# cielavenir/7bgzf

Measured on AMD Instinct MI355X. Metric: GB/s input compressed, BGZF 64KiB blocks, higher is better.
Workload: dtype u8

## Files before the change

### 7bgzf_amd/__init__.py

```python
import ctypes
import os

import numpy as np

HERE = os.path.dirname(os.path.abspath(__file__))
LIB_PATH = os.path.join(HERE, "libhipdeflate.so")

FRAME_RAW, FRAME_BGZF, FRAME_MIGZ, FRAME_RAW_FLUSH, FRAME_ZLIB, FRAME_GZIP = 0, 1, 2, 3, 4, 5
FRAME_LATENCY = 0x100
DEFLATE_HIP = 11
HD_E_NODEVICE, HD_E_ARG, HD_E_NOMEM = 100, 101, 102

BGZF_BLOCK = 0xff00
WG_LEVEL = 3
BGZF_EOF = bytes.fromhex("1f8b08040000000000ff0600424302001b0003000000000000000000")


class HipDeflateError(RuntimeError):
    pass


_lib = None
_vp = ctypes.c_void_p


class MemberSummary(ctypes.Structure):
    _fields_ = [("nmembers", ctypes.c_uint64), ("out_bytes", ctypes.c_uint64), ("end_offset", ctypes.c_uint64),
                ("status", ctypes.c_uint32)]


class RangeSummary(ctypes.Structure):
    _fields_ = [("out_bytes", ctypes.c_uint64), ("nselected", ctypes.c_uint64), ("sel_bytes", ctypes.c_uint64),
                ("nrefused", ctypes.c_uint64), ("bad_member", ctypes.c_uint64), ("status", ctypes.c_uint32)]


RANGE_BYTES, RANGE_VOFFSET = 0, 1
RANGE_PIECE = 256 << 10


def voffset(coffset, uoffset):
    return (int(coffset) << 16) | (int(uoffset) & 0xffff)


EXPORTS = [
    "hipdeflate_init", "hipdeflate_shutdown", "hipdeflate_available", "hipdeflate_version", "hipdeflate_stall_count",
    "hip_deflate", "hip_deflate_flush", "hip_inflate", "hipdeflate_batch_deflate", "hipdeflate_batch_inflate",
    "hipdeflate_batch_deflate_dev", "hipdeflate_batch_inflate_dev", "hipdeflate_scan_sizes_dev",
    "hipdeflate_compact_dev", "hipdeflate_scratch_bytes", "bgzf_compress", "hipdeflate_selftest",
    "hipdeflate_pipe_open", "hipdeflate_pipe_input", "hipdeflate_pipe_submit", "hipdeflate_pipe_result",
    "hipdeflate_pipe_close", "hipdeflate_unpipe_open", "hipdeflate_unpipe_input", "hipdeflate_unpipe_submit",
    "hipdeflate_unpipe_result", "hipdeflate_unpipe_close", "hipdeflate_test_build_lengths", "hipdeflate_test_beside",
    "hip_inflate_flush", "hipdeflate_batch_inflate_flush", "hipdeflate_batch_inflate_flush_dev", "hipdeflate_bound",
    "hipdeflate_compact_span_dev", "hipdeflate_index_members_dev", "hipdeflate_verify_members_dev",
    "hipdeflate_read_ranges_dev",
    "hipdeflate_init_devices", "hipdeflate_device_count", "hipdeflate_use_device",
    "hipdeflate_pipe_open_on", "hipdeflate_unpipe_open_on", "hipdeflate_lat_open_on",
    "hipdeflate_pipe_members", "hipdeflate_lat_open", "hipdeflate_lat_input", "hipdeflate_lat_run", "hipdeflate_lat_output", "hipdeflate_lat_close",
]


def _link_hip_runtime():
    import importlib.util
    spec = importlib.util.find_spec("torch")
    link = os.path.join(HERE, "hiprt", "libamdhip64.so.7")
    target = None
    if spec is not None and spec.submodule_search_locations:
        cand = os.path.join(list(spec.submodule_search_locations)[0], "lib", "libamdhip64.so")
        if os.path.exists(cand):
            target = cand
    try:
        if target is None:
            if os.path.islink(link) or os.path.exists(link):
                os.remove(link)
        elif not (os.path.islink(link) and os.readlink(link) == target):
            os.makedirs(os.path.dirname(link), exist_ok=True)
            if os.path.islink(link) or os.path.exists(link):
                os.remove(link)
            os.symlink(target, link)
    except OSError:
        pass


def lib():
    global _lib
# ... 41 lines not shown
                                               ctypes.POINTER(MemberSummary), _vp]
    L.hipdeflate_verify_members_dev.argtypes = [_vp, _vp, _vp, _vp, _vp, ctypes.c_uint32, ctypes.POINTER(ctypes.c_uint64), _vp]
    L.hipdeflate_read_ranges_dev.argtypes = [_vp, _vp, _vp, _vp, _vp, _vp, ctypes.c_uint32, ctypes.c_int, _vp, _vp, ctypes.c_uint32,
                                             _vp, ctypes.c_uint64, _vp, _vp, _vp, ctypes.POINTER(RangeSummary), _vp]
    L.hipdeflate_pipe_open.restype = _vp
    L.hipdeflate_pipe_open.argtypes = [ctypes.c_int, ctypes.c_int, ctypes.c_uint32, ctypes.c_uint32, ctypes.c_int]
    L.hipdeflate_pipe_input.restype = _vp
    L.hipdeflate_pipe_input.argtypes = [_vp, sz_p]
    L.hipdeflate_pipe_submit.argtypes = [_vp, ctypes.c_size_t]
    L.hipdeflate_pipe_result.argtypes = [_vp, ctypes.POINTER(_vp), sz_p, ctypes.POINTER(ctypes.c_uint32)]
    L.hipdeflate_pipe_members.argtypes = [_vp, ctypes.POINTER(_vp), ctypes.POINTER(_vp), ctypes.POINTER(_vp)]
    L.hipdeflate_pipe_close.restype = None
    L.hipdeflate_pipe_close.argtypes = [_vp]
    L.hipdeflate_unpipe_open.restype = _vp
    L.hipdeflate_unpipe_open.argtypes = [ctypes.c_uint32, ctypes.c_size_t, ctypes.c_size_t, ctypes.c_int]
    L.hipdeflate_unpipe_input.restype = _vp
    L.hipdeflate_unpipe_input.argtypes = [_vp, sz_p]
    L.hipdeflate_unpipe_submit.argtypes = [_vp, _vp, _vp, _vp, ctypes.c_uint32]
    L.hipdeflate_unpipe_result.argtypes = [_vp, ctypes.POINTER(_vp), sz_p]
    L.hipdeflate_unpipe_close.restype = None
    L.hipdeflate_unpipe_close.argtypes = [_vp]
    L.hipdeflate_lat_open.restype = _vp
    L.hipdeflate_lat_open.argtypes = [ctypes.c_int, ctypes.c_int, ctypes.c_uint32, ctypes.c_uint32]
    L.hipdeflate_lat_input.restype = _vp
    L.hipdeflate_lat_input.argtypes = [_vp, ctypes.c_uint32]
    L.hipdeflate_lat_run.argtypes = [_vp, _vp, ctypes.c_uint32]
    L.hipdeflate_lat_output.restype = _vp
    L.hipdeflate_lat_output.argtypes = [_vp, ctypes.c_uint32, _vp, _vp, _vp]
    L.hipdeflate_lat_close.restype = None
    L.hipdeflate_lat_close.argtypes = [_vp]
    L.hipdeflate_test_build_lengths.argtypes = [_vp, ctypes.c_uint32, ctypes.c_uint32, ctypes.c_uint32, _vp]
    L.hipdeflate_test_beside.argtypes = [ctypes.c_int, ctypes.c_uint32]
    L.hipdeflate_test_beside.restype = None
    _lib = L
    return L


def _check(rc, what):
    if rc:
        raise HipDeflateError("%s failed with %d%s" % (
            what, rc, " (no usable gfx950 device; there is no CPU fallback)" if rc == HD_E_NODEVICE else ""))


def available():
    return lib().hipdeflate_available() == 0


def version():
    lib().hipdeflate_available()
    return lib().hipdeflate_version().decode()


def _np(a, dtype):
    return np.ascontiguousarray(a, dtype=dtype)


def _p(a):
    return a.ctypes.data_as(_vp)


def as_u8(data):
    if isinstance(data, np.ndarray):
        return np.ascontiguousarray(data, dtype=np.uint8)
    return np.frombuffer(bytes(data), dtype=np.uint8) if len(data) else np.zeros(0, dtype=np.uint8)


# ... 223 lines not shown
```

### 7bgzf_amd/csrc/hd_api.hip

```cpp
#include <hip/hip_runtime.h>
#include <stdio.h>
#include <stdlib.h>
#include <string.h>
#include <linux/futex.h>
#include <sys/syscall.h>
#include <unistd.h>
#include <sched.h>
#include <chrono>
#include <condition_variable>
#include <mutex>
#include <vector>

#include "../../include/hipdeflate.h"
#include "hd_deflate_static.hpp"
#include "hd_deflate_dynamic.hpp"
#include "hd_deflate_wg.hpp"
#include "hd_emit_wg.hpp"
#include "hd_inflate.hpp"
#include "hd_inflate_lat.hpp"
#include "hd_compact.hpp"
#include "hd_index.hpp"
#include "hd_range.hpp"
#include "hd_segment.hpp"

// ... 58 lines not shown
		const int r = reserve(n);
		if (r) {
			p = old;
			cap = old_cap;
			return r;
		}
		if (old)
			retired.push_back(old);
		return r;
	}
};

struct Ctx {
	bool ready = false;
	int failed = 0;
	int device = -1;
	char desc[256] = "hipdeflate (not initialised)";
	hipStream_t stream = nullptr;
	CrcTables *d_ct = nullptr;
	uint32_t *d_stalls = nullptr;
	std::mutex mu;
	Buf d_in, d_meta, d_slots, d_packed, d_scratch, d_scan;
	Buf h_in{ nullptr, 0, true }, h_meta{ nullptr, 0, true }, h_out{ nullptr, 0, true };
	std::mutex mu_dev;
	Buf d_tok;
	Buf d_tiles;
	hipEvent_t ev_tok = nullptr;
	hipStream_t st_tok = nullptr;
	bool tok_used = false;
	hd::WgBeside beside;
	hipEvent_t ev_tiles = nullptr;
	hipStream_t st_tiles = nullptr;
	bool tiles_used = false;
	std::mutex mu_index;
	Buf d_index, d_cand;
	Buf d_range, d_range_out;
};

constexpr int HD_MAX_CTX = 32;
Ctx g_all[HD_MAX_CTX];
int g_want[HD_MAX_CTX];
int g_nctx = 0;
thread_local int t_cur = 0;
std::mutex g_init_mu;
inline Ctx &cur() { return g_all[t_cur]; }

}
int hd_probe_lds_order(void);
namespace {
constexpr int CODEC_LEVELS = 13;
constexpr size_t CODEC_POOL_MAX = 64;
std::mutex g_codec_mu;
std::vector<hipdeflate_lat *> g_codec_free[CODEC_LEVELS];
void codec_pool_drain()
{
	std::lock_guard<std::mutex> lk(g_codec_mu);
	for (std::vector<hipdeflate_lat *> &f : g_codec_free) {
		for (hipdeflate_lat *c : f)
			hipdeflate_lat_close(c);
		f.clear();
	}
}

void build_crc_tables(CrcTables *t)
{
	const uint32_t poly = 0xEDB88320u;
// ... 138 lines not shown
	stamp();
	if (e != hipSuccess || ndev == 0) {
		fprintf(stderr, "hipdeflate: no HIP device (%s); there is no CPU fallback\n",
			e == hipSuccess ? "device count 0" : hipGetErrorString(e));
		return g.failed = HD_E_NODEVICE;
	}
	if (device < 0) {
		const char *s = getenv("HIPDEFLATE_DEVICE");
		if (!s || !*s)
			s = getenv("LOCAL_RANK");
		device = s && *s ? atoi(s) % ndev : 0;
	}
	if (device >= ndev)
		device = device % ndev;
	hipDeviceProp_t prop;
	HD_CHECK(hipSetDevice(device));
	HD_CHECK(hipGetDeviceProperties(&prop, device));
	if (strncmp(prop.gcnArchName, "gfx950", 6) != 0) {
		fprintf(stderr, "hipdeflate: device %d is %s; this library holds gfx950 (MI355X) code only\n", device,
			prop.gcnArchName);
		return g.failed = HD_E_NODEVICE;
	}
	stamp();
	HD_CHECK(hipStreamCreateWithFlags(&g.stream, hipStreamNonBlocking));
	stamp();
	CrcTables *h = (CrcTables *)malloc(sizeof(CrcTables));
	build_crc_tables(h);
	stamp();
	HD_CHECK(hipMalloc((void **)&g.d_ct, sizeof(CrcTables)));
	HD_CHECK(hipMemcpy(g.d_ct, h, sizeof(CrcTables), hipMemcpyHostToDevice));
	free(h);
	HD_CHECK(hipMalloc((void **)&g.d_stalls, 16));
	HD_CHECK(hipMemset(g.d_stalls, 0, 16));
	stamp();
	if (const int bad = hd_probe_lds_order()) {
		fprintf(stderr, "hipdeflate: device %d failed the LDS store-order probe (%d); this build's encoders are not "
			"reproducible on it and refuse to run\n", device, bad);
		(void)hipFree(g.d_ct);
		g.d_ct = nullptr;
		(void)hipFree(g.d_stalls);
		g.d_stalls = nullptr;
		(void)hipStreamDestroy(g.stream);
		g.stream = nullptr;
		return g.failed = HD_E_NODEVICE;
	}
	stamp();
	if (trace && nts == 7)
		fprintf(stderr, "hipdeflate init (ms): runtime + device count %.1f, set device + properties %.1f, stream %.1f, CRC tables on the CPU %.1f, "
			"first allocations + copy %.1f, first kernel (code object load + LDS order probe) %.1f; total %.1f\n",
			ts[1] - ts[0], ts[2] - ts[1], ts[3] - ts[2], ts[4] - ts[3], ts[5] - ts[4], ts[6] - ts[5], ts[6] - ts[0]);
	g.device = device;
	snprintf(g.desc, sizeof(g.desc), "hipdeflate 0.2 on device %d: %s (%s), %d CUs, %.0f GiB", device, prop.name,
		 prop.gcnArchName, prop.multiProcessorCount, prop.totalGlobalMem / 1073741824.0);
	g.ready = true;
	return 0;
}

inline int ensure_ctx(int idx)
{
	Ctx &g = g_all[idx];
	if (g.ready)
		return 0;
	{
		std::lock_guard<std::mutex> lk(g_init_mu);
		configure_locked(nullptr, 0);
		if (idx >= g_nctx)
			return HD_E_ARG;
	}
	return ctx_init(g, g_want[idx]);
}
inline int ensure() { return ensure_ctx(t_cur); }

inline int bind_device(const Ctx &g)
{
	HD_CHECK(hipSetDevice(g.device));
	return 0;
}
inline int bind_device() { return bind_device(cur()); }

struct OnCtx {
	int keep;
	explicit OnCtx(int idx) : keep(t_cur) { t_cur = idx; }
	~OnCtx() { t_cur = keep; }
};

static int code_batch(const hd::DeflateArgs &a, int level, hipStream_t st)
{
	if (level <= 1) {
		hd::DeflateArgs b = a;
		b.level = level;
		if (a.seg_slots)
			hipLaunchKernelGGL((hd::k_deflate_static<HD_L1_WIN_BITS, HD_L1_HASH_BITS, false, 0, true>), dim3(a.nblocks),
					   dim3(64), 0, st, b);
		else
			hipLaunchKernelGGL((hd::k_deflate_static<HD_L1_WIN_BITS, HD_L1_HASH_BITS, false>), dim3(a.nblocks), dim3(64), 0, st, b);
		return 0;
	}
	return hd::launch_deflate_dynamic(a, level, st);
}

int launch_deflate(const hd::DeflateArgs &a, int level, hipStream_t st)
{
	if (a.nblocks == 0)
		return 0;
	int r = a.seg_limit
			? hd::launch_deflate_segmented(a, level, st, [&](const hd::DeflateArgs &x) { return code_batch(x, level, st); })
			: code_batch(a, level, st);
	if (r)
		return r;
	if (a.frame == HD_FRAME_ZLIB)
		hipLaunchKernelGGL(hd::k_adler32_patch, dim3(a.nblocks), dim3(64), 0, st, a.in, a.in_off, a.in_len, a.nblocks,
				   a.out, a.out_stride, a.out_len, a.status);
	HD_CHECK(hipGetLastError());
	return 0;
}

inline size_t up16(size_t v) { return (v + 15) & ~(size_t)15; }

}

extern "C" {

int hipdeflate_init(int device)
{
	{
		std::lock_guard<std::mutex> lk(g_init_mu);
		if (device < 0)
			configure_locked(nullptr, 0);
		else
			configure_locked(&device, 1);
	}
	return ensure();
}

int hipdeflate_init_devices(const int *devices, int n)
{
	if (!devices || n < 1 || n > HD_MAX_CTX)
// ... 44 lines not shown
		Ctx &g = g_all[i];
		if (!g.ready || !g.d_stalls)
			continue;
		uint32_t v = 0;
		if (hipSetDevice(g.device) == hipSuccess && hipDeviceSynchronize() == hipSuccess &&
		    hipMemcpy(&v, g.d_stalls, 4, hipMemcpyDeviceToHost) == hipSuccess)
			sum += v;
	}
	return sum;
}

const char *hipdeflate_version(void) { return cur().desc; }

static void infb_drain();

void hipdeflate_shutdown(void)
{
	codec_pool_drain();
	infb_drain();
	std::lock_guard<std::mutex> lk(g_init_mu);
	for (int i = 0; i < HD_MAX_CTX; i++) {
		Ctx &g = g_all[i];
		g.failed = 0;
		if (!g.ready)
			continue;
		(void)hipSetDevice(g.device);
		(void)hipDeviceSynchronize();
		for (Buf *b : { &g.d_in, &g.d_meta, &g.d_slots, &g.d_packed, &g.d_scratch, &g.d_scan, &g.h_in, &g.h_meta,
				&g.h_out, &g.d_tok, &g.d_tiles, &g.d_index, &g.d_cand, &g.d_range, &g.d_range_out })
			b->release();
		(void)hipFree(g.d_ct);
		(void)hipFree(g.d_stalls);
		g.d_stalls = nullptr;
		(void)hipStreamDestroy(g.stream);
		if (g.ev_tok)
			(void)hipEventDestroy(g.ev_tok);
		if (g.ev_tiles)
			(void)hipEventDestroy(g.ev_tiles);
		g.ev_tok = g.ev_tiles = nullptr;
		g.beside.release();
		g.st_tok = g.st_tiles = nullptr;
		g.tok_used = g.tiles_used = false;
		g.d_ct = nullptr;
		g.stream = nullptr;
		g.ready = false;
	}
	g_nctx = 0;
}

static uint64_t scratch_need(uint32_t nblocks, uint32_t cap, int level, bool latency)
{
	if (level >= 1 && level < HD_WG_LEVEL && latency && cap > HD_LAT_SEG_BYTES(level))
		return hd::segmented_scratch_bytes(nblocks, cap, level, HD_LAT_SEG_BYTES(level));
	if (level >= 1 && level < HD_WG_LEVEL && cap > HD_SEG_LIMIT)
		return hd::segmented_scratch_bytes(nblocks, cap, level);
	return level < 2 ? 0 : hd::dynamic_scratch_bytes(nblocks, cap, level, 0, latency);
}

uint64_t hipdeflate_scratch_bytes(uint32_t nblocks, uint32_t max_block, int level)
{
	return scratch_need(nblocks, max_block, level, false);
}

uint64_t hipdeflate_bound(uint64_t block_bytes, int level)
{
	const uint32_t lat = HD_LAT_SEG_BYTES(level);
// ... 46 lines not shown
	a.skip_small = 0;
	a.split_max = hd::split_max_block(out_stride, out_cap);
	a.split_ovf = nullptr;
	const uint32_t seg_lim = latency ? HD_LAT_SEG_BYTES(level) : HD_SEG_LIMIT;
	a.seg_bytes = latency ? HD_LAT_SEG_BYTES(level) : HD_SEG_BYTES;
	a.seg_limit = (level >= 1 && level < HD_WG_LEVEL && a.split_max > seg_lim) ? seg_lim : 0;
	if (level >= HD_WG_LEVEL && max_in)
		a.split_max = max_in;
	a.lat = (latency && level >= HD_WG_LEVEL && a.split_max <= hd::EW_BLOCK_MAX) ? 1u : 0u;
	a.stalls = g.d_stalls;
	a.hint = 0;
	a.host_seg_off = nullptr;
	a.host_seg_len = nullptr;
	const uint64_t need = scratch_need(nblocks, a.split_max, level, latency);
	if (need) {
		std::lock_guard<std::mutex> lk(g.mu_dev);
		bool beside_fits = true;
		if (g.d_tok.grow_keep_old(need)) {
			const uint64_t extra = (level >= HD_WG_LEVEL && !a.lat) ? hd::wg_beside_bytes(nblocks, a.split_max) : 0;
			if (!extra || extra >= need || g.d_tok.grow_keep_old(need - extra))
				return HD_E_NOMEM;
			beside_fits = false;
		}
		a.scratch = (uint8_t *)g.d_tok.p;
		if (!g.ev_tok)
			HD_CHECK(hipEventCreateWithFlags(&g.ev_tok, hipEventDisableTiming));
		if (g.tok_used && g.st_tok != (hipStream_t)stream)
			HD_CHECK(hipStreamWaitEvent((hipStream_t)stream, g.ev_tok, 0));
		if (level >= HD_WG_LEVEL && !a.lat && beside_fits && beside_allowed() && g.beside.init() == 0) {
			a.beside = &g.beside;
			const uint32_t keep = (HD_WG_WAYS(level) == 4 && a.split_max <= 65536) ? 2u : 3u;
			a.beside_keep = g_test_beside_keep < keep ? g_test_beside_keep : keep;
		}
		r = launch_deflate(a, level, (hipStream_t)stream);
		if (!r) {
			HD_CHECK(hipEventRecord(g.ev_tok, (hipStream_t)stream));
			g.st_tok = (hipStream_t)stream;
			g.tok_used = true;
		}
		return r;
	}
	return launch_deflate(a, level, (hipStream_t)stream);
}

int hipdeflate_batch_deflate_dev(const void *in, const void *in_off, const void *in_len, uint32_t nblocks, int level,
				 int frame, void *out, uint64_t out_stride, uint32_t out_cap, void *out_len,
				 void *crc32, void *status, void *stream)
{
	return batch_deflate_dev_impl(in, in_off, in_len, nblocks, level, frame, out, out_stride, out_cap, out_len, crc32, status,
				      stream, 0);
}

static int batch_inflate_dev(const void *in, const void *in_off, const void *in_len, uint32_t nblocks, void *out,
			     const void *out_off, const void *out_cap, void *out_len, void *crc32, void *status, void *stream,
			     uint32_t flags)
{
	Ctx &g = cur();
	int r = ensure();
	if (r)
		return r;
	if (!out_len)
		return HD_E_ARG;
	if (nblocks == 0)
		return 0;
	hd::InflateArgs a;
	a.in = (const uint8_t *)in;
	a.in_off = (const uint64_t *)in_off;
	a.in_len = (const uint32_t *)in_len;
	a.nblocks = nblocks;
	a.out = (uint8_t *)out;
	a.out_off = (const uint64_t *)out_off;
	a.out_cap = (const uint32_t *)out_cap;
	a.out_len = (uint32_t *)out_len;
	a.crc = (uint32_t *)crc32;
	a.status = (int32_t *)status;
// ... 25 lines not shown
	Ctx &g = cur();
	int r = ensure();
	if (r)
		return r;
	if (nblocks == 0) {
		if (total)
			HD_CHECK(hipMemsetAsync(total, 0, 8, (hipStream_t)stream));
		return 0;
	}
	const uint32_t ntiles = (nblocks + hd::SCAN_TILE - 1) / hd::SCAN_TILE;
	std::lock_guard<std::mutex> lk(g.mu_dev);
	if (g.d_tiles.grow_keep_old((size_t)ntiles * 8))
		return HD_E_NOMEM;
	uint64_t *tiles = (uint64_t *)g.d_tiles.p;
	hipStream_t st = (hipStream_t)stream;
	if (!g.ev_tiles)
		HD_CHECK(hipEventCreateWithFlags(&g.ev_tiles, hipEventDisableTiming));
	if (g.tiles_used && g.st_tiles != st)
		HD_CHECK(hipStreamWaitEvent(st, g.ev_tiles, 0));
	hipLaunchKernelGGL(hd::k_scan_tile_sums, dim3(ntiles), dim3(256), 0, st, (const uint32_t *)out_len, nblocks, tiles);
	hipLaunchKernelGGL(hd::k_scan_tiles, dim3(1), dim3(256), 0, st, tiles, ntiles, base, (uint64_t *)total);
	hipLaunchKernelGGL(hd::k_scan_finish, dim3(ntiles), dim3(256), 0, st, (const uint32_t *)out_len, nblocks, tiles,
			   (uint64_t *)dst_off);
	HD_CHECK(hipGetLastError());
	HD_CHECK(hipEventRecord(g.ev_tiles, st));
	g.st_tiles = st;
	g.tiles_used = true;
	return 0;
}

int hipdeflate_compact_dev(const void *slots, uint64_t stride, const void *out_len, const void *dst_off,
			   uint32_t nblocks, void *dst, void *stream)
{
	int r = ensure();
	if (r)
		return r;
	if (nblocks == 0)
		return 0;
	if ((stride & 3) || ((uintptr_t)slots & 3))
		return HD_E_ARG;
	hd::launch_compact((const uint8_t *)slots, stride, (const uint32_t *)out_len, (const uint64_t *)dst_off, nblocks,
			   (uint8_t *)dst, (hipStream_t)stream);
	HD_CHECK(hipGetLastError());
	return 0;
}

int hipdeflate_compact_span_dev(const void *slots, uint64_t stride, const void *out_len, const void *dst_off,
				uint32_t nblocks, void *span, uint64_t span_base, void *stream)
{
	return hipdeflate_compact_dev(slots, stride, out_len, dst_off, nblocks, (uint8_t *)span - span_base, stream);
}


static void index_scan(const uint32_t *len, uint32_t n, uint64_t *tiles, uint64_t *dst, uint64_t *total, hipStream_t st)
{
	const uint32_t ntiles = (n + hd::SCAN_TILE - 1) / hd::SCAN_TILE;
	hipLaunchKernelGGL(hd::k_scan_tile_sums, dim3(ntiles), dim3(256), 0, st, len, n, tiles);
	hipLaunchKernelGGL(hd::k_scan_tiles, dim3(1), dim3(256), 0, st, tiles, ntiles, (uint64_t)0, total);
	hipLaunchKernelGGL(hd::k_scan_finish, dim3(ntiles), dim3(256), 0, st, len, n, tiles, dst);
}

int hipdeflate_index_members_dev(const void *blob, uint64_t nbytes, uint32_t max_members, void *in_off, void *in_len,
				 void *out_size, void *out_off, void *crc_want, hipdeflate_member_summary *summary, void *stream)
{
	Ctx &g = cur();
	int r = ensure();
	if (r)
		return r;
	if (!summary || ((uintptr_t)blob & 15) || (nbytes && !blob))
		return HD_E_ARG;
	memset(summary, 0, sizeof *summary);
	if (nbytes == 0)
		return 0;
	hipStream_t st = (hipStream_t)stream;
	const uint8_t *src = (const uint8_t *)blob;
	std::lock_guard<std::mutex> lk(g.mu_index);
// ... 920 lines not shown
	a.in_off = d_off;
	a.in_len = d_len;
	a.nblocks = n;
	a.frame = frame;
	a.level = c->level;
	a.out = c->dout;
	a.out_stride = c->slot;
	a.out_cap = out_cap < c->slot ? out_cap : c->slot;
	a.out_len = d_olen;
	a.crc = d_crc;
	a.status = d_st;
	a.ct = g.d_ct;
	a.scratch = (uint8_t *)c->d_scratch.p;
	a.first = 0;
	a.count = 0;
	a.skip_small = 0;
	a.split_max = c->level >= HD_WG_LEVEL ? c->in_stride : hd::split_max_block(c->slot, c->slot);
	a.split_ovf = nullptr;
	a.seg_bytes = c->seg;
	a.seg_limit = seg_limit;
	a.lat = (latency && c->level >= HD_WG_LEVEL && a.split_max <= hd::EW_BLOCK_MAX) ? 1u : 0u;
	a.stalls = g.d_stalls;
	a.hint = seg_limit ? hint : 0;
	a.host_seg_off = seg_limit ? (const uint64_t *)(c->dmeta + c->meta_seg) : nullptr;
	a.host_seg_len = seg_limit ? (const uint32_t *)((const uint64_t *)(c->dmeta + c->meta_seg) + (size_t)mb * c->S) : nullptr;
	static const bool poll_on = [] { const char *e = getenv("HIPDEFLATE_LAT_POLL"); return e && *e && *e != '0'; }();
	const bool poll = poll_on && seg_limit && c->S <= 64 && !(a.hint & hd::HD_HINT_NO_SEG);
	volatile uint32_t *flag = (volatile uint32_t *)((uint8_t *)c->h_meta.p + c->flag_off);
	if (poll) {
		a.done_flag = (uint32_t *)(c->dmeta + c->flag_off);
		a.done_count = (uint32_t *)c->d_count.p;
		a.done_epoch = ++c->epoch ? c->epoch : ++c->epoch;
	}
	if ((r = launch_deflate(a, c->level, c->st)))
		return r;
	if (poll) {
		const auto t0 = std::chrono::steady_clock::now();
		for (uint32_t spins = 0; __atomic_load_n((const uint32_t *)flag, __ATOMIC_ACQUIRE) != a.done_epoch; spins++) {
			__builtin_ia32_pause();
			if ((spins & 4095) == 4095 && std::chrono::steady_clock::now() - t0 > std::chrono::milliseconds(50)) {
				HD_CHECK(hipStreamSynchronize(c->st));
				break;
			}
		}
		return 0;
	}
	HD_CHECK(hipStreamSynchronize(c->st));
	return 0;
}

int hipdeflate_lat_run(hipdeflate_lat *c, const uint32_t *in_len, uint32_t n)
{
	return c ? lat_run_ex(c, in_len, n, c->frame, c->latency, c->slot) : HD_E_ARG;
}

const uint8_t *hipdeflate_lat_output(hipdeflate_lat *c, uint32_t i, uint32_t *out_len, uint32_t *crc32, int32_t *status)
{
	if (!c || i >= c->max_blocks)
		return nullptr;
	const uint32_t mb = c->max_blocks;
	const uint32_t *h_olen = (const uint32_t *)((const uint64_t *)c->h_meta.p + mb) + mb;
	if (out_len)
		*out_len = h_olen[i];
	if (crc32)
		*crc32 = h_olen[mb + i];
	if (status)
		*status = (int32_t)h_olen[2 * mb + i];
// ... 402 lines not shown
			}
		}
	}
	const int rc = b->rc, nb = b->n;
	int ret = rc;
	if (!rc) {
		const int32_t st = b->status()[idx];
		const uint32_t olen = b->out_len()[idx];
		if (st) {
			ret = st;
		} else {
			if (olen)
				memcpy(dest, (const uint8_t *)b->h_out.p + my_out, olen);
			*destLen = olen;
		}
	}
	const bool last = __atomic_add_fetch(&b->taken, 1, __ATOMIC_ACQ_REL) == nb;
	lk.lock();
	g_inf_active--;
	if (last) {
		__atomic_store_n(&b->state, 0u, __ATOMIC_RELEASE);
		g_inf_free.notify_all();
	}
	lk.unlock();
	return ret;
}

void hipdeflate_test_beside(int keep, uint32_t sub_cap)
{
	g_test_beside_keep = keep < 0 ? 0u : (uint32_t)keep > hd::BESIDE_KEEP_MAX ? hd::BESIDE_KEEP_MAX : (uint32_t)keep;
	hd::wg_sub_test() = sub_cap;
}

#ifdef HD_EMIT_STATS
int hipdeflate_test_emit_stats(uint64_t *out16)
{
	HD_CHECK(hipDeviceSynchronize());
	HD_CHECK(hipMemcpyFromSymbol(out16, HIP_SYMBOL(hd::g_emit_stats), 128));
	return 0;
}
int hipdeflate_test_emit_stats32(uint64_t *out32)
{
	HD_CHECK(hipDeviceSynchronize());
	HD_CHECK(hipMemcpyFromSymbol(out32, HIP_SYMBOL(hd::g_emit_stats), 256));
	return 0;
}
#endif

#ifdef HD_CLOCK_STAMPS
int hipdeflate_test_clock_marks(uint64_t *out16)
{
	HD_CHECK(hipDeviceSynchronize());
	HD_CHECK(hipMemcpyFromSymbol(out16, HIP_SYMBOL(hd::g_clk_mark), 128));
	static const uint64_t zero[16] = { 0 };
	HD_CHECK(hipMemcpyToSymbol(HIP_SYMBOL(hd::g_clk_mark), zero, 128));
	return 0;
}
int hipdeflate_test_clock(uint64_t *out16)
{
	HD_CHECK(hipDeviceSynchronize());
	HD_CHECK(hipMemcpyFromSymbol(out16, HIP_SYMBOL(hd::g_clk), 128));
	static const uint64_t zero[16] = { 0 };
	HD_CHECK(hipMemcpyToSymbol(HIP_SYMBOL(hd::g_clk), zero, 128));
	return 0;
}
#endif
// ... 34 lines not shown
```

### 7bgzf_amd/csrc/hd_compact.hpp

```cpp
#pragma once
#include "hd_device.hpp"
#include <atomic>

namespace hd {

constexpr uint32_t SCAN_TILE = 2048;

__global__ __launch_bounds__(256) void k_scan_tile_sums(const uint32_t *len, uint32_t n, uint64_t *tile_sum)
{
	__shared__ uint64_t wsum[4];
	const uint32_t t = threadIdx.x, tile = blockIdx.x;
	uint64_t s = 0;
	for (uint32_t i = tile * SCAN_TILE + t; i < n && i < (tile + 1) * SCAN_TILE; i += 256)
		s += len[i];
	for (int o = 32; o > 0; o >>= 1) {
		s += ((uint64_t)(uint32_t)__shfl_down((int)(uint32_t)s, o, 64)) |
		     ((uint64_t)(uint32_t)__shfl_down((int)(uint32_t)(s >> 32), o, 64) << 32);
	}
	if ((t & 63) == 0)
		wsum[t >> 6] = s;
	__syncthreads();
	if (t == 0)
		tile_sum[tile] = wsum[0] + wsum[1] + wsum[2] + wsum[3];
}
// ... 136 lines not shown
	const bool edge = lane < 16 ? lane < head : lane < 32 && lane - 16 < L - done;
	uint8_t eb = 0;
	if (edge)
		eb = s[eo];
	const uint8_t *sb = s + head + 16 * lane;
	uint8_t *db = d + head + 16 * lane;
	uint32_t k = 0;
	for (; k + 64 * U <= lines; k += 64 * U) {
		compact_u32x4 v[U];
#pragma unroll
		for (uint32_t j = 0; j < U; j++)
			v[j] = compact_ld16<NT>(sb + 16 * (k + 64 * j));
#pragma unroll
		for (uint32_t j = 0; j < U; j++)
			compact_st16<NT>(db + 16 * (k + 64 * j), v[j]);
	}
	if (k < lines) {
		compact_u32x4 v[U];
		uint32_t q[U];
#pragma unroll
		for (uint32_t j = 0; j < U; j++) {
			q[j] = k + 64 * j + lane;
			v[j] = compact_ld16<NT>(s + head + 16 * (uint64_t)(q[j] < lines ? q[j] : lines - 1));
		}
#pragma unroll
		for (uint32_t j = 0; j < U; j++)
			if (q[j] < lines)
				compact_st16<NT>(d + head + 16 * (uint64_t)q[j], v[j]);
	}
	if (edge)
		d[eo] = eb;
}

__global__ __launch_bounds__(64) void k_compact(const uint8_t *__restrict__ slots, uint64_t stride, const uint32_t *__restrict__ len,
						const uint64_t *__restrict__ dst_off, uint32_t n, uint8_t *__restrict__ dst)
{
	const uint32_t lane = threadIdx.x, step = gridDim.x;
	uint32_t i = blockIdx.x;
	if (i >= n)
		return;
	uint32_t L = len[i];
	uint64_t o = dst_off[i];
	for (;;) {
		const uint32_t nx = i + step;
		const bool more = nx < n && nx > i;
		const uint32_t nc = more ? nx : i;
		const uint32_t Ln = len[nc];
		const uint64_t on = dst_off[nc];
		compact_wide<COMPACT_NT, COMPACT_UNROLL>(slots + (uint64_t)i * stride, L, dst + o, lane);
		if (!more)
			break;
		i = nx;
		L = Ln;
		o = on;
	}
}

inline uint32_t compact_device_cus()
{
	static std::atomic<uint32_t> cus[64];
	int dev = 0;
	if (hipGetDevice(&dev) != hipSuccess || dev < 0 || dev >= 64)
		return 256;
	uint32_t c = cus[dev].load(std::memory_order_relaxed);
	if (!c) {
		int v = 0;
		if (hipDeviceGetAttribute(&v, hipDeviceAttributeMultiprocessorCount, dev) != hipSuccess || v <= 0)
			v = 256;
		cus[dev].store(c = (uint32_t)v, std::memory_order_relaxed);
	}
	return c;
}

inline void launch_compact(const uint8_t *slots, uint64_t stride, const uint32_t *len, const uint64_t *dst_off, uint32_t n,
			   uint8_t *dst, hipStream_t st)
{
	const uint64_t cap = (uint64_t)compact_device_cus() * COMPACT_WAVES_PER_CU;
	hipLaunchKernelGGL(k_compact, dim3(n < cap ? n : (uint32_t)cap), dim3(64), 0, st, slots, stride, len, dst_off, n, dst);
}

__global__ __launch_bounds__(64) void k_adler32_patch(const uint8_t *in, const uint64_t *in_off, const uint32_t *in_len,
						      uint32_t nblocks, uint8_t *out, uint64_t out_stride,
						      const uint32_t *out_len, const int32_t *status)
{
	const uint32_t b = blockIdx.x, lane = threadIdx.x;
	if (b >= nblocks || (status && status[b]) || out_len[b] < 6)
		return;
	const uint8_t *src = in + in_off[b];
	const uint32_t n = in_len[b];
	const bool aligned = (((uintptr_t)src) & 15) == 0;
	AdlerLanes adl;
	adl.init();
	for (uint32_t piece = 0; piece * HD_PIECE < n; piece++) {
		const uint32_t o = piece * HD_PIECE + lane * 16;
		uint4 v = make_uint4(0, 0, 0, 0);
		if (aligned && o + 16 <= n) {
			v = *(const uint4 *)(src + o);
		} else if (o < n) {
			uint32_t w[4] = { 0, 0, 0, 0 };
#pragma unroll
			for (uint32_t k = 0; k < 16; k++)
				w[k >> 2] |= (o + k < n ? (uint32_t)src[o + k] : 0u) << (8 * (k & 3));
			v = make_uint4(w[0], w[1], w[2], w[3]);
		}
		adl.fold(piece, lane, v);
	}
	const uint32_t a = adl.finish(n);
	if (lane < 4)
		out[(uint64_t)b * out_stride + out_len[b] - 4 + lane] = (uint8_t)(a >> (24 - 8 * lane));
}

// ... 2 lines not shown
```

### 7bgzf_amd/csrc/hd_segment.hpp

```cpp
#pragma once
#include "hd_compact.hpp"
#include "hd_deflate_dynamic.hpp"

namespace hd {

__host__ __device__ inline uint32_t seg_stride(uint32_t seg) { return (HD_STORED_SIZE(seg) + 5u + 32u + 15u) & ~15u; }
constexpr uint32_t SEG_ROUND_MAX = 65536;

struct SegArgs {
	DeflateArgs a;
	uint32_t first, count;
	uint32_t S;
	uint32_t seg, limit;
	uint64_t *seg_off;
	uint32_t *seg_len;
	uint32_t *seg_olen;
	uint32_t *seg_crc;
	int32_t *seg_st;
	uint64_t *seg_dst;
};

inline uint32_t seg_round_blocks(uint32_t nblocks, uint32_t S)
{
	uint32_t r = SEG_ROUND_MAX / S;
// ... 244 lines not shown
		const uint32_t ns = g.count * S;
		if (a.host_seg_off && rb >= a.nblocks) {
			g.seg_off = (uint64_t *)a.host_seg_off;
			g.seg_len = (uint32_t *)a.host_seg_len;
		} else {
			hipLaunchKernelGGL(k_seg_table, dim3((ns + 255) / 256), dim3(256), 0, st, g);
		}
		DeflateArgs s = a;
		s.in_off = g.seg_off;
		s.in_len = g.seg_len;
		s.nblocks = ns;
		s.frame = HD_FRAME_RAW_FLUSH;
		s.out = slots;
		s.out_stride = stride;
		s.out_cap = stride;
		s.out_len = g.seg_olen;
		s.crc = g.seg_crc;
		s.status = g.seg_st;
		s.scratch = inner;
		s.split_max = stride;
		s.seg_limit = 0;
		s.parts = HD_LAT_PARTS(level, seg);
		s.seg_slots = seg != HD_SEG_BYTES ? S : 0;
		if ((r = code(s)))
			return r;
		if (S <= 64) {
			SegArgs gr = g;
			if (first + rb < a.nblocks)
				gr.a.done_flag = nullptr;
			hipLaunchKernelGGL(k_seg_finish, dim3(ns), dim3(64), 0, st, gr, (const uint8_t *)slots, stride);
		} else {
			hipLaunchKernelGGL(k_seg_stitch, dim3(g.count), dim3(64), 0, st, g);
			launch_compact((const uint8_t *)slots, (uint64_t)stride, (const uint32_t *)g.seg_olen,
				       (const uint64_t *)g.seg_dst, ns, a.out, st);
		}
	}
	return 0;
}

}
```

### include/hipdeflate.h

```cpp
#ifndef HIPDEFLATE_H
#define HIPDEFLATE_H

#include <stddef.h>
#include <stdint.h>

#ifdef __cplusplus
extern "C" {
#endif

#define DEFLATE_HIP 11

#define HD_E_NODEVICE  100
#define HD_E_ARG       101
#define HD_E_NOMEM     102

#define HD_FRAME_RAW   0
#define HD_FRAME_BGZF  1
#define HD_FRAME_MIGZ  2
#define HD_FRAME_RAW_FLUSH 3
#define HD_FRAME_ZLIB  4
#define HD_FRAME_GZIP  5

#define HD_FRAME_LATENCY 0x100

// ... 110 lines not shown
			   uint32_t *nblocks);
int hipdeflate_pipe_members(hipdeflate_pipe *p, const uint32_t **out_len, const uint64_t **dst_off,
			    const uint32_t **crc32);
#define HIPDEFLATE_VOFFSET(coffset, uoffset) (((uint64_t)(coffset) << 16) | (uint64_t)((uoffset) & 0xffff))
void hipdeflate_pipe_close(hipdeflate_pipe *p);
hipdeflate_pipe *hipdeflate_pipe_open_on(int index, int level, int frame, uint32_t block_bytes,
					 uint32_t blocks_per_batch, int depth);

typedef struct hipdeflate_unpipe hipdeflate_unpipe;
hipdeflate_unpipe *hipdeflate_unpipe_open(uint32_t max_members, size_t in_cap, size_t out_cap, int depth);
uint8_t *hipdeflate_unpipe_input(hipdeflate_unpipe *p, size_t *cap);
int hipdeflate_unpipe_submit(hipdeflate_unpipe *p, const uint64_t *in_off, const uint32_t *in_len,
			     const uint32_t *out_size, uint32_t nmembers);
int hipdeflate_unpipe_result(hipdeflate_unpipe *p, const uint8_t **data, size_t *nbytes);
void hipdeflate_unpipe_close(hipdeflate_unpipe *p);
hipdeflate_unpipe *hipdeflate_unpipe_open_on(int index, uint32_t max_members, size_t in_cap, size_t out_cap, int depth);

typedef struct hipdeflate_lat hipdeflate_lat;
hipdeflate_lat *hipdeflate_lat_open(int level, int frame, uint32_t max_blocks, uint32_t max_block_bytes);
uint8_t *hipdeflate_lat_input(hipdeflate_lat *c, uint32_t i);
int hipdeflate_lat_run(hipdeflate_lat *c, const uint32_t *in_len, uint32_t n);
const uint8_t *hipdeflate_lat_output(hipdeflate_lat *c, uint32_t i, uint32_t *out_len, uint32_t *crc32, int32_t *status);
void hipdeflate_lat_close(hipdeflate_lat *c);
hipdeflate_lat *hipdeflate_lat_open_on(int index, int level, int frame, uint32_t max_blocks, uint32_t max_block_bytes);

uint64_t hipdeflate_scratch_bytes(uint32_t nblocks, uint32_t max_block, int level);

int bgzf_compress(void *dst, size_t *dlen, const void *src, size_t slen, int level);

int hipdeflate_selftest(void);
int hipdeflate_test_build_lengths(const uint32_t *freq, uint32_t nvec, uint32_t nsyms, uint32_t maxbits,
				  uint8_t *lens_out);
void hipdeflate_test_beside(int keep, uint32_t sub_cap);

#ifdef __cplusplus
}
#endif
#endif
```

Baseline: 376.6.

## Make compact kernel yield to concurrent deflate via device mark and ticket queue

Adds a device-side 'mark' counter that deflate launches raise and lower around large batches. The compact kernel becomes persistent and pulls runs of members from an atomic ticket. When the mark is up, wavefronts above a quiet threshold sleep so a concurrently running deflate on another stream gets the CUs. The intent is to overlap compaction with encoding across streams without starving the encoder. In exchange it adds extra tiny kernel launches, a memset, event waits on a ring of tickets, and spin-sleep polling of global memory.

Result: faster. 384.8, median of 6 (+2.2%).

```diff
diff --git a/7bgzf_amd/__init__.py b/7bgzf_amd/__init__.py
--- a/7bgzf_amd/__init__.py
+++ b/7bgzf_amd/__init__.py
@@ -50,6 +50,7 @@
     "hipdeflate_pipe_open", "hipdeflate_pipe_input", "hipdeflate_pipe_submit", "hipdeflate_pipe_result",
     "hipdeflate_pipe_close", "hipdeflate_unpipe_open", "hipdeflate_unpipe_input", "hipdeflate_unpipe_submit",
     "hipdeflate_unpipe_result", "hipdeflate_unpipe_close", "hipdeflate_test_build_lengths", "hipdeflate_test_beside",
+    "hipdeflate_test_mark_read", "hipdeflate_test_mark_add",
     "hip_inflate_flush", "hipdeflate_batch_inflate_flush", "hipdeflate_batch_inflate_flush_dev", "hipdeflate_bound",
     "hipdeflate_compact_span_dev", "hipdeflate_index_members_dev", "hipdeflate_verify_members_dev",
     "hipdeflate_read_ranges_dev",
@@ -157,6 +158,8 @@
     L.hipdeflate_test_build_lengths.argtypes = [_vp, ctypes.c_uint32, ctypes.c_uint32, ctypes.c_uint32, _vp]
     L.hipdeflate_test_beside.argtypes = [ctypes.c_int, ctypes.c_uint32]
     L.hipdeflate_test_beside.restype = None
+    L.hipdeflate_test_mark_read.argtypes = [_vp, _vp]
+    L.hipdeflate_test_mark_add.argtypes = [ctypes.c_int, _vp]
     _lib = L
     return L
 
diff --git a/7bgzf_amd/csrc/hd_api.hip b/7bgzf_amd/csrc/hd_api.hip
--- a/7bgzf_amd/csrc/hd_api.hip
+++ b/7bgzf_amd/csrc/hd_api.hip
@@ -114,6 +114,13 @@
 	hipEvent_t ev_tiles = nullptr;
 	hipStream_t st_tiles = nullptr;
 	bool tiles_used = false;
+	static constexpr uint32_t GATHER_RING = 8, GATHER_LINE = 32;
+	uint32_t *d_gather = nullptr;
+	uint32_t *mark() const { return d_gather; }
+	uint32_t *ticket(uint32_t e) const { return d_gather + (size_t)GATHER_LINE * (1 + e); }
+	hipEvent_t ev_ticket[GATHER_RING] = {};
+	hipStream_t st_ticket[GATHER_RING] = {};
+	uint32_t ticket_next = 0;
 	std::mutex mu_index;
 	Buf d_index, d_cand;
 	Buf d_range, d_range_out;
@@ -318,6 +325,8 @@
 	free(h);
 	HD_CHECK(hipMalloc((void **)&g.d_stalls, 16));
 	HD_CHECK(hipMemset(g.d_stalls, 0, 16));
+	HD_CHECK(hipMalloc((void **)&g.d_gather, (size_t)Ctx::GATHER_LINE * 4 * (1 + Ctx::GATHER_RING)));
+	HD_CHECK(hipMemset(g.d_gather, 0, (size_t)Ctx::GATHER_LINE * 4 * (1 + Ctx::GATHER_RING)));
 	stamp();
 	if (const int bad = hd_probe_lds_order()) {
 		fprintf(stderr, "hipdeflate: device %d failed the LDS store-order probe (%d); this build's encoders are not "
@@ -326,6 +335,8 @@
 		g.d_ct = nullptr;
 		(void)hipFree(g.d_stalls);
 		g.d_stalls = nullptr;
+		(void)hipFree(g.d_gather);
+		g.d_gather = nullptr;
 		(void)hipStreamDestroy(g.stream);
 		g.stream = nullptr;
 		return g.failed = HD_E_NODEVICE;
@@ -385,10 +396,24 @@
 	return hd::launch_deflate_dynamic(a, level, st);
 }
 
-int launch_deflate(const hd::DeflateArgs &a, int level, hipStream_t st)
+int launch_deflate(const hd::DeflateArgs &a, int level, hipStream_t st, uint32_t *mark)
 {
 	if (a.nblocks == 0)
 		return 0;
+	struct Resident {
+		uint32_t *mark;
+		hipStream_t st;
+		Resident(uint32_t *m, hipStream_t s) : mark(m), st(s)
+		{
+			if (mark)
+				hipLaunchKernelGGL(hd::k_mark_add, dim3(1), dim3(64), 0, st, mark, 1);
+		}
+		~Resident()
+		{
+			if (mark)
+				hipLaunchKernelGGL(hd::k_mark_add, dim3(1), dim3(64), 0, st, mark, -1);
+		}
+	} resident(mark && !a.lat && !a.seg_slots && a.nblocks >= hd::compact_grid_waves() ? mark : nullptr, st);
 	int r = a.seg_limit
 			? hd::launch_deflate_segmented(a, level, st, [&](const hd::DeflateArgs &x) { return code_batch(x, level, st); })
 			: code_batch(a, level, st);
@@ -499,6 +524,15 @@
 		(void)hipFree(g.d_ct);
 		(void)hipFree(g.d_stalls);
 		g.d_stalls = nullptr;
+		(void)hipFree(g.d_gather);
+		g.d_gather = nullptr;
+		for (uint32_t e = 0; e < Ctx::GATHER_RING; e++) {
+			if (g.ev_ticket[e])
+				(void)hipEventDestroy(g.ev_ticket[e]);
+			g.ev_ticket[e] = nullptr;
+			g.st_ticket[e] = nullptr;
+		}
+		g.ticket_next = 0;
 		(void)hipStreamDestroy(g.stream);
 		if (g.ev_tok)
 			(void)hipEventDestroy(g.ev_tok);
@@ -611,7 +645,7 @@
 			const uint32_t keep = (HD_WG_WAYS(level) == 4 && a.split_max <= 65536) ? 2u : 3u;
 			a.beside_keep = g_test_beside_keep < keep ? g_test_beside_keep : keep;
 		}
-		r = launch_deflate(a, level, (hipStream_t)stream);
+		r = launch_deflate(a, level, (hipStream_t)stream, latency ? nullptr : g.mark());
 		if (!r) {
 			HD_CHECK(hipEventRecord(g.ev_tok, (hipStream_t)stream));
 			g.st_tok = (hipStream_t)stream;
@@ -619,7 +653,7 @@
 		}
 		return r;
 	}
-	return launch_deflate(a, level, (hipStream_t)stream);
+	return launch_deflate(a, level, (hipStream_t)stream, latency ? nullptr : g.mark());
 }
 
 int hipdeflate_batch_deflate_dev(const void *in, const void *in_off, const void *in_len, uint32_t nblocks, int level,
@@ -711,6 +745,7 @@
 int hipdeflate_compact_dev(const void *slots, uint64_t stride, const void *out_len, const void *dst_off,
 			   uint32_t nblocks, void *dst, void *stream)
 {
+	Ctx &g = cur();
 	int r = ensure();
 	if (r)
 		return r;
@@ -718,9 +753,25 @@
 		return 0;
 	if ((stride & 3) || ((uintptr_t)slots & 3))
 		return HD_E_ARG;
+	hipStream_t st = (hipStream_t)stream;
+	if (nblocks < hd::compact_grid_waves()) {
+		hd::launch_compact((const uint8_t *)slots, stride, (const uint32_t *)out_len, (const uint64_t *)dst_off, nblocks,
+				   (uint8_t *)dst, st, nullptr, nullptr);
+		HD_CHECK(hipGetLastError());
+		return 0;
+	}
+	std::lock_guard<std::mutex> lk(g.mu_dev);
+	const uint32_t e = g.ticket_next;
+	if (!g.ev_ticket[e])
+		HD_CHECK(hipEventCreateWithFlags(&g.ev_ticket[e], hipEventDisableTiming));
+	else if (g.st_ticket[e] != st)
+		HD_CHECK(hipStreamWaitEvent(st, g.ev_ticket[e], 0));
 	hd::launch_compact((const uint8_t *)slots, stride, (const uint32_t *)out_len, (const uint64_t *)dst_off, nblocks,
-			   (uint8_t *)dst, (hipStream_t)stream);
+			   (uint8_t *)dst, st, g.ticket(e), g.mark());
 	HD_CHECK(hipGetLastError());
+	HD_CHECK(hipEventRecord(g.ev_ticket[e], st));
+	g.st_ticket[e] = st;
+	g.ticket_next = (e + 1) % Ctx::GATHER_RING;
 	return 0;
 }
 
@@ -1707,7 +1758,7 @@
 		a.done_count = (uint32_t *)c->d_count.p;
 		a.done_epoch = ++c->epoch ? c->epoch : ++c->epoch;
 	}
-	if ((r = launch_deflate(a, c->level, c->st)))
+	if ((r = launch_deflate(a, c->level, c->st, nullptr)))
 		return r;
 	if (poll) {
 		const auto t0 = std::chrono::steady_clock::now();
@@ -2176,6 +2227,27 @@
 	hd::wg_sub_test() = sub_cap;
 }
 
+int hipdeflate_test_mark_read(void *out, void *stream)
+{
+	Ctx &g = cur();
+	int r = ensure();
+	if (r)
+		return r;
+	HD_CHECK(hipMemcpyAsync(out, g.mark(), 8, hipMemcpyDefault, (hipStream_t)stream));
+	return 0;
+}
+
+int hipdeflate_test_mark_add(int delta, void *stream)
+{
+	Ctx &g = cur();
+	int r = ensure();
+	if (r)
+		return r;
+	hipLaunchKernelGGL(hd::k_mark_add, dim3(1), dim3(64), 0, (hipStream_t)stream, g.mark(), delta);
+	HD_CHECK(hipGetLastError());
+	return 0;
+}
+
 #ifdef HD_EMIT_STATS
 int hipdeflate_test_emit_stats(uint64_t *out16)
 {
diff --git a/7bgzf_amd/csrc/hd_compact.hpp b/7bgzf_amd/csrc/hd_compact.hpp
--- a/7bgzf_amd/csrc/hd_compact.hpp
+++ b/7bgzf_amd/csrc/hd_compact.hpp
@@ -192,27 +192,81 @@
 		d[eo] = eb;
 }
 
+#ifndef HD_COMPACT_QUIET_WAVES
+#define HD_COMPACT_QUIET_WAVES 128
+#endif
+#ifndef HD_COMPACT_SLEEP
+#define HD_COMPACT_SLEEP 8
+#endif
+#ifndef HD_COMPACT_RUN
+#define HD_COMPACT_RUN 4
+#endif
+constexpr uint32_t COMPACT_QUIET_WAVES = HD_COMPACT_QUIET_WAVES;
+constexpr uint32_t COMPACT_SLEEP = HD_COMPACT_SLEEP;
+constexpr uint32_t COMPACT_RUN = HD_COMPACT_RUN;
+constexpr uint32_t COMPACT_RUNS_EACH = 8;
+static_assert(COMPACT_QUIET_WAVES >= 1, "somebody has to copy while the mark is up");
+static_assert(COMPACT_SLEEP >= 1, "a yielding wavefront that does not sleep polls the L2 without a pause");
+static_assert(COMPACT_RUN >= 1 && COMPACT_RUN <= 64 && COMPACT_RUNS_EACH >= 1, "a run is a handful of members");
+
+__device__ __forceinline__ uint32_t compact_word(const uint32_t *p)
+{
+	return (uint32_t)__builtin_amdgcn_readfirstlane((int)__hip_atomic_load(p, __ATOMIC_RELAXED, __HIP_MEMORY_SCOPE_AGENT));
+}
+
 __global__ __launch_bounds__(64) void k_compact(const uint8_t *__restrict__ slots, uint64_t stride, const uint32_t *__restrict__ len,
-						const uint64_t *__restrict__ dst_off, uint32_t n, uint8_t *__restrict__ dst)
-{
-	const uint32_t lane = threadIdx.x, step = gridDim.x;
-	uint32_t i = blockIdx.x;
-	if (i >= n)
-		return;
-	uint32_t L = len[i];
-	uint64_t o = dst_off[i];
+						const uint64_t *__restrict__ dst_off, uint32_t n, uint8_t *__restrict__ dst,
+						uint32_t *ticket, const uint32_t *mark, uint32_t run)
+{
+	const uint32_t lane = threadIdx.x;
+	const bool yields = ticket && mark && blockIdx.x >= COMPACT_QUIET_WAVES;
+	const uint32_t nruns = ticket ? (n - 1) / run + 1 : 0;
+	uint32_t m = 1;
 	for (;;) {
-		const uint32_t nx = i + step;
-		const bool more = nx < n && nx > i;
-		const uint32_t nc = more ? nx : i;
-		const uint32_t Ln = len[nc];
-		const uint64_t on = dst_off[nc];
-		compact_wide<COMPACT_NT, COMPACT_UNROLL>(slots + (uint64_t)i * stride, L, dst + o, lane);
-		if (!more)
-			break;
-		i = nx;
-		L = Ln;
-		o = on;
+		uint32_t i = blockIdx.x, e = i + 1;
+		if (ticket) {
+			if (yields && m) {
+				while (compact_word(mark)) {
+					if (compact_word(ticket) >= nruns)
+						return;
+#pragma unroll
+					for (uint32_t k = 0; k < COMPACT_SLEEP; k++)
+						__builtin_amdgcn_s_sleep(127);
+				}
+			}
+			uint32_t mv = 0, t = 0;
+			if (yields)
+				mv = __hip_atomic_load(mark, __ATOMIC_RELAXED, __HIP_MEMORY_SCOPE_AGENT);
+			if (lane == 0)
+				t = __hip_atomic_fetch_add(ticket, 1u, __ATOMIC_RELAXED, __HIP_MEMORY_SCOPE_AGENT);
+			t = (uint32_t)__builtin_amdgcn_readfirstlane((int)t);
+			m = (uint32_t)__builtin_amdgcn_readfirstlane((int)mv);
+			if (t >= nruns)
+				return;
+			i = t * run;
+			e = n - i < run ? n : i + run;
+		}
+		if (i >= n)
+			return;
+		uint32_t L = len[i];
+		uint64_t o = dst_off[i];
+		for (;;) {
+			const bool more = i + 1 < e;
+			const uint32_t nc = more ? i + 1 : i;
+			const uint32_t Ln = len[nc];
+			const uint64_t on = dst_off[nc];
+			const uint64_t so = (uint64_t)i * stride;
+			const uint32_t so_lo = (uint32_t)__builtin_amdgcn_readfirstlane((int)(uint32_t)so);
+			const uint32_t so_hi = (uint32_t)__builtin_amdgcn_readfirstlane((int)(uint32_t)(so >> 32));
+			compact_wide<COMPACT_NT, COMPACT_UNROLL>(slots + (((uint64_t)so_hi << 32) | so_lo), L, dst + o, lane);
+			if (!more)
+				break;
+			i = nc;
+			L = Ln;
+			o = on;
+		}
+		if (!ticket)
+			return;
 	}
 }
 
@@ -232,11 +286,34 @@
 	return c;
 }
 
+inline uint32_t compact_grid_waves()
+{
+	return compact_device_cus() * COMPACT_WAVES_PER_CU;
+}
+
+__global__ __launch_bounds__(64) void k_mark_add(uint32_t *mark, int32_t delta)
+{
+	if (threadIdx.x == 0) {
+		(void)__hip_atomic_fetch_add(mark, (uint32_t)delta, __ATOMIC_RELAXED, __HIP_MEMORY_SCOPE_AGENT);
+		if (delta > 0)
+			(void)__hip_atomic_fetch_add(mark + 1, 1u, __ATOMIC_RELAXED, __HIP_MEMORY_SCOPE_AGENT);
+	}
+}
+
 inline void launch_compact(const uint8_t *slots, uint64_t stride, const uint32_t *len, const uint64_t *dst_off, uint32_t n,
-			   uint8_t *dst, hipStream_t st)
-{
-	const uint64_t cap = (uint64_t)compact_device_cus() * COMPACT_WAVES_PER_CU;
-	hipLaunchKernelGGL(k_compact, dim3(n < cap ? n : (uint32_t)cap), dim3(64), 0, st, slots, stride, len, dst_off, n, dst);
+			   uint8_t *dst, hipStream_t st, uint32_t *ticket, const uint32_t *mark)
+{
+	const uint32_t cap = compact_grid_waves();
+	if (n < cap || !ticket) {
+		hipLaunchKernelGGL(k_compact, dim3(n), dim3(64), 0, st, slots, stride, len, dst_off, n, dst, (uint32_t *)nullptr,
+				   (const uint32_t *)nullptr, 1u);
+		return;
+	}
+	if (hipMemsetAsync(ticket, 0, 4, st) != hipSuccess)
+		return;
+	const uint32_t each = n / (cap * COMPACT_RUNS_EACH);
+	hipLaunchKernelGGL(k_compact, dim3(cap), dim3(64), 0, st, slots, stride, len, dst_off, n, dst, ticket, mark,
+			   n > 0x80000000u && COMPACT_RUN < 2 ? 2u : each < 1 ? 1u : each < COMPACT_RUN ? each : COMPACT_RUN);
 }
 
 __global__ __launch_bounds__(64) void k_adler32_patch(const uint8_t *in, const uint64_t *in_off, const uint32_t *in_len,
diff --git a/7bgzf_amd/csrc/hd_segment.hpp b/7bgzf_amd/csrc/hd_segment.hpp
--- a/7bgzf_amd/csrc/hd_segment.hpp
+++ b/7bgzf_amd/csrc/hd_segment.hpp
@@ -300,7 +300,7 @@
 		} else {
 			hipLaunchKernelGGL(k_seg_stitch, dim3(g.count), dim3(64), 0, st, g);
 			launch_compact((const uint8_t *)slots, (uint64_t)stride, (const uint32_t *)g.seg_olen,
-				       (const uint64_t *)g.seg_dst, ns, a.out, st);
+				       (const uint64_t *)g.seg_dst, ns, a.out, st, nullptr, nullptr);
 		}
 	}
 	return 0;
diff --git a/include/hipdeflate.h b/include/hipdeflate.h
--- a/include/hipdeflate.h
+++ b/include/hipdeflate.h
@@ -166,6 +166,8 @@
 int hipdeflate_test_build_lengths(const uint32_t *freq, uint32_t nvec, uint32_t nsyms, uint32_t maxbits,
 				  uint8_t *lens_out);
 void hipdeflate_test_beside(int keep, uint32_t sub_cap);
+int hipdeflate_test_mark_read(void *out, void *stream);
+int hipdeflate_test_mark_add(int delta, void *stream);
 
 #ifdef __cplusplus
 }
```
